# Chang-Tun-Yu/HLS-final-Visual-Odometry

Measured on AMD Instinct MI355X. Metric: stereo frame-pairs/sec (detect+match), KITTI 1241x376; matches bit-exact, higher is better.
Workload: dtype u8; 1 GPU; KITTI 1241x376 stereo quad-match (prev/curr x L/R), default 50x50 bins; noise=0, gpu_max_hw_queues=4, streams_per_gpu=256, frames_in_hbm=8, parallelism=1x independent stream groups

## Files before the change

hls-final-visual-odometry_amd/csrc/kernels_detect.hip:

```cpp
#include "vh_dev.h"
#include "vh_wave.h"
#include <type_traits>

namespace {

__global__ void half_res_kernel(VhImages src, uint8_t *__restrict__ dst, VhGeom g) {
  const int32_t id = blockIdx.z;
  const uint8_t *__restrict__ I = vh_image_ptr(src, id);
  uint8_t *__restrict__ O = dst + (int64_t)id * g.bplm * g.Hm;
  const int32_t u = blockIdx.x * blockDim.x + threadIdx.x;
  const int32_t v = blockIdx.y;
  if (u >= g.bplm) return;
  uint32_t val = 0;
  if (u < g.Wm) {
    const int64_t r0 = (int64_t)(2 * v) * g.bpl + 2 * u, r1 = r0 + g.bpl;
    val = ((uint32_t)I[r0] + I[r0 + 1] + I[r1] + I[r1 + 1]) >> 2;
  }
  O[(int64_t)v * g.bplm + u] = (uint8_t)val;
}

__global__ void __launch_bounds__(256)
detect_nms_kernel(VhImages im, VhGeom g, uint64_t *__restrict__ rec, int32_t *__restrict__ chunk_count) {
  extern __shared__ __attribute__((aligned(16))) uint8_t smem[];
  uint8_t *sI = smem;
  int16_t *sF1 = (int16_t *)(smem + (size_t)g.IH * g.IWp);
  int16_t *sF2 = sF1 + (size_t)g.FH * g.FWp;

  const int32_t id = blockIdx.z;
  const uint8_t *__restrict__ I = vh_image_ptr(im, id);
  const int32_t n = g.n, n1 = n + 1;
  const int32_t bx0 = blockIdx.x * g.tbx, by0 = blockIdx.y * g.tby;
  const int32_t fx0 = VH_MARGIN + bx0 * n1, fy0 = VH_MARGIN + by0 * n1;
  const int32_t ix0 = fx0 - 2, iy0 = fy0 - 2;
  const int32_t tid = threadIdx.x;

  for (int32_t k = tid; k < g.IH * g.IWp; k += 256) {
    const int32_t r = k / g.IWp, c = k - r * g.IWp;
    const int32_t gx = ix0 + c, gy = iy0 + r;
    uint8_t v = 0;
    if (c < g.IW && gx < g.bplm && gy < g.Hm) v = I[(int64_t)gy * g.bplm + gx];
    sI[k] = v;
  }
  __syncthreads();

  {
    const int32_t nseg = max(1, 256 / g.FW);
    const int32_t rows_per = (g.FH + nseg - 1) / nseg;
    for (int32_t task = tid; task < g.FW * nseg; task += 256) {
      const int32_t seg = task / g.FW, cx = task - seg * g.FW;
      const int32_t r0 = seg * rows_per, r1 = min(g.FH, r0 + rows_per);
      if (r0 >= r1) continue;
      int32_t h5[5], h3[5], hc[5], cc[5];
#pragma unroll
      for (int32_t k = 0; k < 4; k++) {
        const uint8_t *p = sI + (size_t)(r0 + k) * g.IWp + cx;
        const int32_t a = p[0], b = p[1], c = p[2], d = p[3], e = p[4];
        h5[k + 1] = a + b + c + d + e; h3[k + 1] = b + c + d; hc[k + 1] = a + b - d - e; cc[k + 1] = c;
      }
      for (int32_t fr = r0; fr < r1; fr++) {
#pragma unroll
        for (int32_t k = 0; k < 4; k++) { h5[k] = h5[k + 1]; h3[k] = h3[k + 1]; hc[k] = hc[k + 1]; cc[k] = cc[k + 1]; }
        const uint8_t *p = sI + (size_t)(fr + 4) * g.IWp + cx;
        const int32_t a = p[0], b = p[1], c = p[2], d = p[3], e = p[4];
        h5[4] = a + b + c + d + e; h3[4] = b + c + d; hc[4] = a + b - d - e; cc[4] = c;
        const int32_t f2 = hc[0] + hc[1] - hc[3] - hc[4];
        const int32_t f1 = -(h5[0] + h5[1] + h5[2] + h5[3] + h5[4]) + 2 * (h3[1] + h3[2] + h3[3]) + 7 * cc[2];
        sF1[(size_t)fr * g.FWp + cx] = (int16_t)f1;
        sF2[(size_t)fr * g.FWp + cx] = (int16_t)f2;
      }
    }
  }
  __syncthreads();

  int32_t *sCnt = (int32_t *)(sF2 + (size_t)g.FH * g.FWp);
  uint32_t *sWork = (uint32_t *)(sCnt + 1);
  uint16_t *sCode = (uint16_t *)(sWork + 4 * g.tbx * g.tby);
  const int32_t nblk_tile = g.tbx * g.tby;
  if (tid == 0) *sCnt = 0;
  for (int32_t k = tid; k < 4 * nblk_tile; k += 256) sCode[k] = VH_NO_CODE;
  __syncthreads();
  const int32_t xlim = (g.Wm - 1 - VH_MARGIN) - fx0, ylim = (g.Hm - 1 - VH_MARGIN) - fy0;
  const int32_t lby = tid / g.tbx, lbx = tid - lby * g.tbx;
  const int32_t bx = bx0 + lbx, by = by0 + lby;
  const bool have_block = tid < nblk_tile && bx < g.nbx && by < g.nby;
  if (have_block) {
    const int32_t fx = n + lbx * n1, fy = n + lby * n1;
    int32_t ex[4], ey[4], ev[4];
    ex[0] = ex[1] = ex[2] = ex[3] = fx;
    ey[0] = ey[1] = ey[2] = ey[3] = fy;
    ev[0] = ev[1] = sF1[(size_t)fy * g.FWp + fx];
    ev[2] = ev[3] = sF2[(size_t)fy * g.FWp + fx];
    for (int32_t j2 = fy; j2 <= fy + n; j2++) {
      for (int32_t i2 = fx; i2 <= fx + n; i2++) {
        int32_t cur = sF1[(size_t)j2 * g.FWp + i2];
        if (cur < ev[0]) { ex[0] = i2; ey[0] = j2; ev[0] = cur; }
        else if (cur > ev[1]) { ex[1] = i2; ey[1] = j2; ev[1] = cur; }
        cur = sF2[(size_t)j2 * g.FWp + i2];
        if (cur < ev[2]) { ex[2] = i2; ey[2] = j2; ev[2] = cur; }
        else if (cur > ev[3]) { ex[3] = i2; ey[3] = j2; ev[3] = cur; }
      }
    }
#pragma unroll
    for (int32_t c = 0; c < 4; c++) {
      const bool pass = (c & 1) ? (ev[c] >= g.tau) : (ev[c] <= -g.tau);
      if (pass) sWork[atomicAdd(sCnt, 1)] = (uint32_t)ex[c] | ((uint32_t)ey[c] << 10) | ((uint32_t)c << 20) | ((uint32_t)tid << 22);
    }
  }
  __syncthreads();
  const int32_t nwork = *sCnt;
  for (int32_t w = tid; w < nwork; w += 256) {
    const uint32_t e = sWork[w];
    const int32_t cx = e & 1023, cy = (e >> 10) & 1023, c = (e >> 20) & 3, owner = e >> 22;
    const int32_t oby = owner / g.tbx, obx = owner - oby * g.tbx;
    const int32_t fx = n + obx * n1, fy = n + oby * n1;
    const int16_t *F = (c < 2) ? sF1 : sF2;
    const bool is_min = (c & 1) == 0;
    const int32_t val = F[(size_t)cy * g.FWp + cx];
    const int32_t jhi = min(cy + n, ylim), ihi = min(cx + n, xlim);
    bool ok = true;
    for (int32_t j2 = cy - n; j2 <= jhi && ok; j2++) {
      for (int32_t i2 = cx - n; i2 <= ihi; i2++) {
        const int32_t cur = F[(size_t)j2 * g.FWp + i2];
        const bool outside = (i2 < fx) | (i2 > fx + n) | (j2 < fy) | (j2 > fy + n);
        if (outside && (is_min ? (cur < val) : (cur > val))) { ok = false; break; }
      }
    }
    if (ok) sCode[owner * 4 + c] = (uint16_t)(((cy - fy) << 6) | (cx - fx));
  }
  __syncthreads();
  if (have_block) {
    uint64_t code = 0;
    int32_t cnt = 0;
#pragma unroll
    for (int32_t c = 0; c < 4; c++) {
      const uint32_t pc = sCode[tid * 4 + c];
      code |= (uint64_t)pc << (16 * c);
      cnt += pc != VH_NO_CODE ? 1 : 0;
    }
    const int32_t blk = by * g.nbx + bx;
    rec[(int64_t)id * g.nblocks + blk] = code;
    if (cnt) atomicAdd(&chunk_count[(int64_t)id * g.nchunks + blk / VH_CHUNK], cnt);
  }
}

#ifdef VH_EMIT_TIMING
__device__ unsigned long long g_emit_t[8];
extern "C" int32_t vh_debug_emit_timing(unsigned long long *out, int32_t reset) {
  if (hipMemcpyFromSymbol(out, HIP_SYMBOL(g_emit_t), sizeof(g_emit_t)) != hipSuccess) return -3;
  if (reset) { unsigned long long z[8] = {0}; z[6] = ~0ull; if (hipMemcpyToSymbol(HIP_SYMBOL(g_emit_t), z, sizeof(z)) != hipSuccess) return -3; }
  return 0;
}
#define VH_TICK_IMPL(k) do { __syncthreads(); if (t_on_) { const unsigned long long now_ = __builtin_readcyclecounter(); atomicAdd(&g_emit_t[k], now_ - t_prev_); t_prev_ = now_; if ((k) == 4) atomicMax(&g_emit_t[7], now_); } } while (0)
#define VH_TICK_INIT_IMPL const bool t_on_ = threadIdx.x == 0 && (blockIdx.x + gridDim.x * (blockIdx.y + gridDim.y * blockIdx.z)) % 61 == 0; unsigned long long t_prev_ = __builtin_readcyclecounter(); if (t_on_) { atomicAdd(&g_emit_t[5], 1ull); atomicMin(&g_emit_t[6], t_prev_); }
#endif
#if defined(VH_EMIT_TIMING) && VH_EMIT_TIMING == 2
#define VH_DTICK(k) VH_TICK_IMPL(k)
#define VH_DTICK_INIT VH_TICK_INIT_IMPL
#else
#define VH_DTICK(k) do { } while (0)
#define VH_DTICK_INIT do { } while (0)
#endif
#if defined(VH_EMIT_TIMING) && VH_EMIT_TIMING != 2
#define VH_ETICK(k) VH_TICK_IMPL(k)
#define VH_ETICK_INIT VH_TICK_INIT_IMPL
#else
#define VH_ETICK(k) do { } while (0)
#define VH_ETICK_INIT do { } while (0)
#endif

#ifdef VH_EXP_DET_STOP
#define VH_DET_STOP(k)                                                                                   \
  if (VH_EXP_DET_STOP == (k) && g.nbx > 0) {                                                              \
    const int32_t sbx = bx0 + tid % T::TBX, sby = by0 + tid / T::TBX;                                     \
    if (sbx < g.nbx && sby < g.nby) rec[(int64_t)id * g.nblocks + sby * g.nbx + sbx] = ~0ull;              \
    return;                                                                                               \
  }
#else
#define VH_DET_STOP(k) do { } while (0)
#endif

template <int N> struct DetTile {
  static constexpr int N1 = N + 1, TBX = 32, TBY = 8;
  static constexpr int FW = TBX * N1 + 2 * N, FH = TBY * N1 + 2 * N;
  static constexpr int IW = FW + 4, IH = FH + 4;
  static constexpr int OFF = (VH_MARGIN - 2) & 3;
  static constexpr int DW = ((IW + 3 + 3) / 4 + 3) / 4 * 4;
  static constexpr int IP = DW * 4;
  static constexpr int NC = DW / 4;
  static constexpr int groups(int px) { return (FW + OFF + px - 1) / px; }
  static constexpr int seg_cost(int px, int s) {
    const int rows = (FH + s - 1) / s, waves = (groups(px) * s + 63) / 64;
    const int hrow = px == 4 ? 28 : 18, vrow = px == 4 ? 26 : 13;
    return groups(px) * s > 256 || rows * (s - 1) >= FH ? (1 << 30) : 1000 * ((rows + 4) * hrow + rows * vrow) + waves;
  }
  static constexpr int best_seg(int px) {
    int b = 1;
    for (int s = 2; s <= 16; s++)
      if (seg_cost(px, s) < seg_cost(px, b)) b = s;
    return b;
  }
#ifdef VH_DET_PX
  static constexpr int PX = VH_DET_PX;
  static constexpr int SEG = VH_DET_SEG;
#else
  static constexpr int PX = seg_cost(2, best_seg(2)) < seg_cost(4, best_seg(4)) ? 2 : 4;
  static constexpr int SEG = best_seg(PX);
#endif
  static constexpr int G = groups(PX);
  static constexpr int FP = PX * G;
  static constexpr int ROWS = (FH + SEG - 1) / SEG;
  static constexpr int BIAS = 8192;
  static_assert((G - 1) * PX / 4 + 1 <= DW - 1, "a group reads the staged dword it starts in and the next one");
  static_assert(G * SEG <= 256, "one lane per (group, row segment)");
  static constexpr int LAST = FH - (SEG - 1) * ROWS;
  static_assert(LAST >= 1, "every segment has rows");
};

template <int N>
__global__ void __launch_bounds__(256)
detect_nms_fast_kernel(VhImages im, VhGeom g, uint64_t *__restrict__ rec, int32_t *__restrict__ chunk_count) {
  using T = DetTile<N>;
  constexpr int N1 = T::N1, WN = 2 * N + 1;
  VH_DET_SETPRIO();
  constexpr int X_BYTES = (T::IH * T::IP > 6144) ? T::IH * T::IP : 6144;
  __shared__ __attribute__((aligned(16))) int16_t sF1[T::FH * T::FP];
  __shared__ __attribute__((aligned(16))) int16_t sF2[T::FH * T::FP];
  __shared__ __attribute__((aligned(16))) uint8_t sX[X_BYTES];
  uint8_t *sI = sX;

  const int32_t id = blockIdx.z, tid = threadIdx.x;
  const uint8_t *__restrict__ I = vh_image_ptr(im, id);
  const int32_t bx0 = blockIdx.x * T::TBX, by0 = blockIdx.y * T::TBY;
  const int32_t fx0 = VH_MARGIN + bx0 * N1, fy0 = VH_MARGIN + by0 * N1;
  const int32_t ix0 = fx0 - 2, iy0 = fy0 - 2;
  const int32_t ax0 = ix0 - T::OFF;
  VH_DTICK_INIT;

  {
    constexpr int NLD = (T::IH * T::NC + 255) / 256;
    typedef uint32_t u32x4a4 __attribute__((ext_vector_type(4), aligned(4)));
    typedef uint32_t u32x4 __attribute__((ext_vector_type(4)));
    const uint32_t last = (uint32_t)g.Hm * (uint32_t)g.bplm - 16u;
    u32x4 stg[NLD];
#pragma unroll
    for (int32_t i = 0; i < NLD; i++) {
      const int32_t k = min(tid + 256 * i, T::IH * T::NC - 1);
      const int32_t r = k / T::NC, c = k - r * T::NC;
      stg[i] = *(const u32x4a4 *)(I + min((uint32_t)(iy0 + r) * (uint32_t)g.bplm + (uint32_t)(ax0 + 16 * c), last));
    }
    __builtin_amdgcn_sched_barrier(0);
#pragma unroll
    for (int32_t i = 0; i < NLD; i++) {
      const int32_t k = tid + 256 * i;
      if (k < T::IH * T::NC) ((u32x4 *)sI)[k] = stg[i];
    }
  }
  __syncthreads();

  VH_DTICK(0);
  VH_DET_STOP(1);
  if (tid < T::G * T::SEG) {
    constexpr int PX = T::PX, NR = PX / 2;
    const int32_t seg = tid / T::G, gq = tid - seg * T::G;
    const int32_t r0 = seg * T::ROWS;
    {
      constexpr uint32_t HB = 512u * 0x00010001u, KB = (uint32_t)T::BIAS * 0x00010001u;
      const uint32_t *p = (const uint32_t *)sI + r0 * T::DW + (gq * PX) / 4;
      const uint32_t sel0 = 0x0c010c00u + ((PX == 2 && (gq & 1)) ? 0x00020002u : 0u);
      uint32_t *o1 = (uint32_t *)sF1 + (r0 * T::FP + PX * gq) / 2, *o2 = (uint32_t *)sF2 + (r0 * T::FP + PX * gq) / 2;
      uint32_t h5[NR][5], h3[NR][5], pc[NR][4], cc[NR][5], hcp[NR], S5[NR];
#pragma unroll
      for (int32_t h = 0; h < NR; h++) S5[h] = 0u;
#pragma unroll
      for (int32_t t = 0; t < T::ROWS + 4; t++) {
        if (t - 4 < T::LAST || r0 + t - 4 < T::FH) {
          const uint32_t A = p[t * T::DW], B = p[t * T::DW + 1];
          uint32_t pk[PX + 3];
#pragma unroll
          for (int32_t k = 0; k < PX + 3; k++) pk[k] = __builtin_amdgcn_perm(B, A, sel0 + (uint32_t)k * 0x00010001u);
          uint32_t n5[NR], n3[NR], nc[NR], nz[NR];
          if (PX == 4) {
            const uint32_t a01 = pk[0] + pk[1], a23 = pk[2] + pk[3], a34 = pk[3] + pk[4], a56 = pk[5] + pk[6];
            n3[0] = a23 + pk[1];             n3[NR - 1] = a34 + pk[5];
            n5[0] = n3[0] + pk[0] + pk[4];   n5[NR - 1] = n3[NR - 1] + pk[2] + pk[6];
            nc[0] = (a01 + HB) - a34;        nc[NR - 1] = (a23 + HB) - a56;
            nz[0] = pk[2];                   nz[NR - 1] = pk[4];
          } else {
            n3[0] = pk[1] + pk[2] + pk[3];
            n5[0] = n3[0] + pk[0] + pk[4];
            nc[0] = ((pk[0] + pk[1]) + HB) - (pk[3] + pk[4]);
            nz[0] = pk[2];
          }
          uint32_t f1[NR], f2[NR];
#pragma unroll
          for (int32_t h = 0; h < NR; h++) {
            const uint32_t old5 = h5[h][0];
#pragma unroll
            for (int32_t k = 0; k < 4; k++) { h5[h][k] = h5[h][k + 1]; h3[h][k] = h3[h][k + 1]; cc[h][k] = cc[h][k + 1]; }
            h5[h][4] = n5[h]; h3[h][4] = n3[h]; cc[h][4] = nz[h];
            S5[h] += n5[h];
            if (t >= 5) S5[h] -= old5;
#pragma unroll
            for (int32_t k = 0; k < 3; k++) pc[h][k] = pc[h][k + 1];
            if (t > 0) pc[h][3] = hcp[h] + nc[h];
            hcp[h] = nc[h];
            if (t >= 4) {
              const uint32_t S3 = h3[h][1] + h3[h][2] + h3[h][3];
              f2[h] = (pc[h][0] + KB) - pc[h][3];
              f1[h] = ((S3 + S3) + (__umul24(cc[h][2], 7u) + KB)) - S5[h];
            }
          }
          if (t >= 4) {
            if (PX == 4) {
              *(uint2 *)(o1 + (t - 4) * (T::FP / 2)) = make_uint2(f1[0], f1[NR - 1]);
              *(uint2 *)(o2 + (t - 4) * (T::FP / 2)) = make_uint2(f2[0], f2[NR - 1]);
            } else {
              o1[(t - 4) * (T::FP / 2)] = f1[0];
              o2[(t - 4) * (T::FP / 2)] = f2[0];
            }
          }
        }
      }
    }
  }
  __syncthreads();
  VH_DTICK(1);
  VH_DET_STOP(2);

  const int32_t xlim = min(max((g.Wm - 1 - VH_MARGIN) - fx0, 0), T::FW - 1);
  const int32_t ylim = min(max((g.Hm - 1 - VH_MARGIN) - fy0, 0), T::FH - 1);
  const int32_t lby = tid / T::TBX, lbx = tid % T::TBX;
  const int32_t bx = bx0 + lbx, by = by0 + lby;
  const bool have_block = bx < g.nbx && by < g.nby;
  const int32_t fx = N + lbx * N1, fy = N + lby * N1;
  uint32_t *sQueue = (uint32_t *)sX;
  uint16_t *sCode = (uint16_t *)(sQueue + 1024);
  __shared__ uint32_t sQueueN;
  if (tid == 0) sQueueN = 0;
  ((uint2 *)sCode)[tid] = make_uint2(VH_NO_CODE * 0x00010001u, VH_NO_CODE * 0x00010001u);
  __syncthreads();
  {
    typedef int16_t i16x2 __attribute__((ext_vector_type(2)));
    const int32_t lane = tid & 63;
    bool cand[4];
    uint32_t ext[4];
#pragma unroll
    for (int32_t plane = 0; plane < 2; plane++) {
      const int16_t *b = (plane ? sF2 : sF1) + fy * T::FP + fx + T::OFF;
      int32_t vn, vx;
      if (N & 1) {
        const i16x2 *bw = (const i16x2 *)b;
        i16x2 mn = bw[0], mx = mn;
#pragma unroll
        for (int32_t j = 0; j < N1; j++) {
#pragma unroll
          for (int32_t d = 0; d < N1 / 2; d++) {
            if (d == 0 && j == 0) continue;
            const i16x2 w = bw[j * (T::FP / 2) + d];
            mn = __builtin_elementwise_min(mn, w);
            mx = __builtin_elementwise_max(mx, w);
          }
        }
        vn = min((int32_t)mn.x, (int32_t)mn.y);
        vx = max((int32_t)mx.x, (int32_t)mx.y);
      } else {
        vn = vx = b[0];
#pragma unroll
        for (int32_t k = 1; k < N1 * N1; k++) {
          const int32_t cur = b[(k / N1) * T::FP + k % N1];
          vn = min(vn, cur);
          vx = max(vx, cur);
        }
      }
      cand[2 * plane] = have_block && vn <= T::BIAS - g.tau;
      cand[2 * plane + 1] = have_block && vx >= T::BIAS + g.tau;
      ext[2 * plane] = (uint32_t)vn;
      ext[2 * plane + 1] = (uint32_t)vx;
    }
    uint64_t bal[4];
#pragma unroll
    for (int32_t t = 0; t < 4; t++) bal[t] = __ballot(cand[t]);
    const uint32_t n0 = (uint32_t)__popcll(bal[0]), n1 = (uint32_t)__popcll(bal[1]);
    const uint32_t add = (n0 + (uint32_t)__popcll(bal[2])) | ((n1 + (uint32_t)__popcll(bal[3])) << 16);
    if (add) {
      uint32_t base = 0;
      if (lane == 0) base = atomicAdd(&sQueueN, add);
      base = __builtin_amdgcn_readfirstlane(base);
#pragma unroll
      for (int32_t t = 0; t < 4; t++) {
        const int32_t mm = t & 1;
        const uint32_t first = ((base >> (16 * mm)) & 0xFFFFu) + (t >= 2 ? (mm ? n1 : n0) : 0u);
        const uint32_t rank = (uint32_t)vh_wave_rank(bal[t]);
        if (cand[t]) sQueue[mm * 512 + first + rank] = (uint32_t)tid | ((uint32_t)t << 8) | (ext[t] << 16);
      }
    }
  }
  __syncthreads();
  VH_DTICK(2);
  VH_DET_STOP(3);
  {
    const int32_t n0 = (int32_t)(sQueueN & 0xFFFFu), ntot = n0 + (int32_t)(sQueueN >> 16);
    const bool unclipped = xlim == T::FW - 1 && ylim == T::FH - 1;
    auto check = [&](auto kind, auto no_clip, int32_t e) {
      const uint32_t q = sQueue[e < n0 ? e : 512 + e - n0];
      const int32_t owner = q & 255, type = (q >> 8) & 3;
      const int32_t ofy = N + (owner / T::TBX) * N1, ofx = N + (owner % T::TBX) * N1;
      const int16_t *F = ((type & 2) ? sF2 : sF1) + T::OFF;
      const int32_t val = (int32_t)(q >> 16);
      const int16_t *bb = F + ofy * T::FP + ofx;
      int32_t pos = (N << 6) | N;
#pragma unroll
      for (int32_t idx = N1 * N1 - 2; idx >= 0; idx--)
        pos = bb[(idx / N1) * T::FP + idx % N1] == val ? (((idx / N1) << 6) | (idx % N1)) : pos;
      const int32_t bj = pos >> 6, bi = pos & 63;
      const int32_t cy = ofy + bj, cx = ofx + bi;
      int32_t v[WN * WN];
      if (decltype(no_clip)::value) {
        const int16_t *w = F + (cy - N) * T::FP + (cx - N);
#pragma unroll
        for (int32_t j = 0; j < WN; j++)
#pragma unroll
          for (int32_t k = 0; k < WN; k++) v[j * WN + k] = w[j * T::FP + k];
      } else {
        int32_t col[WN];
#pragma unroll
        for (int32_t k = 0; k < WN; k++) col[k] = min(cx - N + k, xlim);
#pragma unroll
        for (int32_t j = 0; j < WN; j++) {
          const int16_t *row = F + min(cy - N + j, ylim) * T::FP;
#pragma unroll
          for (int32_t k = 0; k < WN; k++) v[j * WN + k] = row[col[k]];
        }
      }
      const int32_t centre = v[N * WN + N];
      int32_t emin = centre, emax = centre;
#pragma unroll
      for (int32_t k = 0; k < WN * WN; k++) {
        if (decltype(kind)::value != 1) emin = min(emin, v[k]);
        if (decltype(kind)::value != 0) emax = max(emax, v[k]);
      }
      const int32_t ext = decltype(kind)::value == 0 ? emin : decltype(kind)::value == 1 ? emax : ((type & 1) ? emax : emin);
      if (ext == centre) sCode[owner * 4 + type] = (uint16_t)((bj << 6) | bi);
    };
    typedef std::integral_constant<int, 0> KMin;
    typedef std::integral_constant<int, 1> KMax;
    typedef std::integral_constant<int, 2> KBoth;
    for (int32_t e = tid; e < ntot; e += 256) {
      const int32_t e0 = __builtin_amdgcn_readfirstlane(e & ~63);
      if (e0 + 63 < n0) { if (unclipped) check(KMin{}, std::true_type{}, e); else check(KMin{}, std::false_type{}, e); }
      else if (e0 >= n0) { if (unclipped) check(KMax{}, std::true_type{}, e); else check(KMax{}, std::false_type{}, e); }
      else { if (unclipped) check(KBoth{}, std::true_type{}, e); else check(KBoth{}, std::false_type{}, e); }
    }
  }
  __syncthreads();
  VH_DTICK(3);
  VH_DET_STOP(4);
  uint32_t codes[4];
  {
    const uint2 cw = ((const uint2 *)sCode)[tid];
    codes[0] = cw.x & 0xFFFFu; codes[1] = cw.x >> 16; codes[2] = cw.y & 0xFFFFu; codes[3] = cw.y >> 16;
  }

  __shared__ int32_t sChunk[16];
  const int32_t chunk_lo = (by0 * g.nbx + bx0) / VH_CHUNK;
  if (tid < 16) sChunk[tid] = 0;
  __syncthreads();
  if (have_block) {
    int32_t cnt = 0;
#pragma unroll
    for (int32_t c = 0; c < 4; c++) cnt += codes[c] != VH_NO_CODE ? 1 : 0;
    const int32_t blk = by * g.nbx + bx;
    rec[(int64_t)id * g.nblocks + blk] = (uint64_t)(codes[0] | (codes[1] << 16)) | ((uint64_t)(codes[2] | (codes[3] << 16)) << 32);
    if (cnt) atomicAdd(&sChunk[blk / VH_CHUNK - chunk_lo], cnt);
  }
  __syncthreads();
  if (tid < 16 && sChunk[tid]) atomicAdd(&chunk_count[(int64_t)id * g.nchunks + chunk_lo + tid], sChunk[tid]);
  VH_DTICK(4);
}

__constant__ int8_t c_desc_dx[16] = {-3, -3, -1, -1, +3, +3, +1, +1, -1, -1, +1, +1, -5, -5, +5, +5};
__constant__ int8_t c_desc_dy[16] = {-1, +1, -1, +1, -1, +1, -1, +1, -5, +5, -5, +5, -3, +3, -3, +3};


#ifndef VH_EMIT_NF
#define VH_EMIT_NF 2
#endif
__global__ void __launch_bounds__(256)
emit_features_kernel(VhImages im, VhGeom g, const uint64_t *__restrict__ rec,
                     const int32_t *__restrict__ chunk_count, VhSets s) {
  int32_t *__restrict__ feat = s.feat;
  int32_t *__restrict__ count = s.count;
  const int32_t cap = s.cap;
  __shared__ uint32_t sList[4 * VH_CHUNK + 1];
  __shared__ int32_t sWave[4], sWaveP[4];

  const int32_t id = blockIdx.y, chunk = blockIdx.x, tid = threadIdx.x;
  const uint8_t *__restrict__ I = vh_image_ptr(im, id);
  const int32_t set = vh_image_set(im, id);
  const int32_t n1 = g.n + 1;
  VH_DET_SETPRIO();
  VH_ETICK_INIT;

  constexpr int BPL = VH_CHUNK / 256;
  uint32_t clo[BPL], chi[BPL];
  {
    const uint2 *rp = reinterpret_cast<const uint2 *>(rec) + (int64_t)id * g.nblocks;
#pragma unroll
    for (int32_t k = 0; k < BPL; k++) {
      const uint2 c = rp[min(chunk * VH_CHUNK + tid * BPL + k, g.nblocks - 1)];
      clo[k] = c.x; chi[k] = c.y;
    }
  }
  int32_t part = 0;
  for (int32_t k = tid; k < chunk; k += 256) part += chunk_count[(int64_t)id * g.nchunks + k];
  int32_t mine = 0;
#pragma unroll
  for (int32_t k = 0; k < BPL; k++) {
    if (chunk * VH_CHUNK + tid * BPL + k >= g.nblocks) clo[k] = chi[k] = ~0u;
    mine += ((clo[k] & 0xFFFFu) != VH_NO_CODE) + ((clo[k] >> 16) != VH_NO_CODE) + ((chi[k] & 0xFFFFu) != VH_NO_CODE) + ((chi[k] >> 16) != VH_NO_CODE);
  }
  part = vh_wave_sum(part);
  const int32_t incl = vh_wave_scan(mine);
  if ((tid & 63) == 63) { sWave[tid >> 6] = incl; sWaveP[tid >> 6] = part; }
  __syncthreads();
  const int32_t base = sWaveP[0] + sWaveP[1] + sWaveP[2] + sWaveP[3];
  VH_ETICK(0);
  int32_t woff = 0;
  for (int32_t w = 0; w < (tid >> 6); w++) woff += sWave[w];
  const int32_t total = sWave[0] + sWave[1] + sWave[2] + sWave[3];
  int32_t pos = woff + incl - mine;
  {
    const int32_t blk0 = chunk * VH_CHUNK + tid * BPL;
    int32_t by = blk0 / g.nbx, bx = blk0 - by * g.nbx;
    const uint32_t org = (uint32_t)(g.n + VH_MARGIN) * ((1u << 14) + 1u);
#pragma unroll
    for (int32_t k = 0; k < BPL; k++) {
      const uint32_t pxy = org + (uint32_t)(bx * n1) + ((uint32_t)(by * n1) << 14);
#pragma unroll
      for (int32_t q = 0; q < 4; q++) {
        const uint32_t w = (q < 2) ? clo[k] : chi[k];
        const uint32_t pc = (q & 1) ? (w >> 16) : (w & 0xFFFFu);
        const bool ok = pc != VH_NO_CODE;
        const uint32_t e = pxy + (pc & 63u) + ((pc >> 6) << 14) + ((uint32_t)q << 28);
        sList[ok ? pos : 4 * VH_CHUNK] = e;
        pos += ok ? 1 : 0;
      }
      if (++bx == g.nbx) { bx = 0; by++; }
    }
  }
  __syncthreads();
  if (chunk == g.nchunks - 1 && tid == 0) count[set] = base + total;
  VH_ETICK(1);
  const int32_t grp = tid >> 4, k = tid & 15;
  const int32_t dx = c_desc_dx[k], dy = c_desc_dy[k];
  constexpr int NF = VH_EMIT_NF;
  const int32_t prk = min(k, 14) - 7;
  typedef uint32_t u32x4a1 __attribute__((ext_vector_type(4), aligned(1)));
  struct Coords { int32_t fs[NF], us[NF], vs[NF], cs[NF]; bool lives[NF]; };
  auto fetch = [&](int32_t f0, Coords &q, u32x4a1 (&prow)[NF]) {
#pragma unroll
    for (int32_t h = 0; h < NF; h++) {
      q.fs[h] = f0 + 16 * h + grp;
      q.lives[h] = q.fs[h] < total;
      const uint32_t e = sList[q.lives[h] ? q.fs[h] : 0];
      q.us[h] = e & 0x3FFF; q.vs[h] = (e >> 14) & 0x3FFF; q.cs[h] = e >> 28;
#ifdef VH_EXP_NOPATCH
      prow[h] = u32x4a1{(uint32_t)q.us[h], (uint32_t)q.vs[h], 0u, 0u};
#else
      prow[h] = *(const u32x4a1 *)(I + (__umul24((uint32_t)(q.vs[h] + prk), (uint32_t)g.bplm) + (uint32_t)(q.us[h] - 7)));
#endif
    }
  };
  Coords qa, qb;
  u32x4a1 pa[NF], pb[NF];
  if (total > 0) fetch(0, qa, pa);

  constexpr int ROWS_LDS = 64;
  __shared__ int32_t sRow[4 * ROWS_LDS];
  __shared__ __attribute__((aligned(16))) uint16_t sLoc[4 * VH_CHUNK];
  const int32_t blk_first = chunk * VH_CHUNK, blk_last = min(blk_first + VH_CHUNK, g.nblocks) - 1;
  const int32_t v_first = ((blk_first / g.nbx) * n1 + g.n + VH_MARGIN) * g.scale;
  const int32_t v_span = ((blk_last / g.nbx) * n1 + g.n + VH_MARGIN + g.n) * g.scale + g.scale - v_first;
  const bool rows_in_lds = v_span <= ROWS_LDS;
  int32_t *__restrict__ rowh = s.row_hist + (int64_t)set * 4 * s.H;
  auto bin_of_entry = [&](uint32_t e) {
    const int32_t uu = (int32_t)(e & 0x3FFF) * g.scale, vv = (int32_t)((e >> 14) & 0x3FFF) * g.scale, c = e >> 28;
    const int32_t ubin = s.binsize == 1 ? uu : (int32_t)__umulhi((uint32_t)uu, s.inv_binsize);
    const int32_t vbin = s.binsize == 1 ? vv : (int32_t)__umulhi((uint32_t)vv, s.inv_binsize);
    return (c * s.ubn + min(ubin, s.ubn - 1)) * s.vbn + min(vbin, s.vbn - 1);
  };
  const bool have0 = tid < total && base + tid < cap;
  const int32_t b0 = have0 ? bin_of_entry(sList[tid]) : 0;
  int32_t slot0 = 0;
  if (have0) slot0 = atomicAdd(&s.hist[(int64_t)set * s.nbins + b0], 1);
  if (rows_in_lds) {
    for (int32_t k = tid; k < 4 * ROWS_LDS; k += 256) sRow[k] = 0;
    __syncthreads();
    for (int32_t f = tid; f < total && base + f < cap; f += 256) {
      const uint32_t e = sList[f];
      const int32_t vv = (int32_t)((e >> 14) & 0x3FFF) * g.scale, c = e >> 28;
      sLoc[f] = (uint16_t)atomicAdd(&sRow[c * ROWS_LDS + (vv - v_first)], 1);
    }
    __syncthreads();
    for (int32_t k = tid; k < 4 * ROWS_LDS; k += 256) {
      const int32_t cnt = sRow[k], c = k / ROWS_LDS, vv = v_first + k % ROWS_LDS;
      if (cnt) sRow[k] = atomicAdd(&rowh[c * s.H + vv], cnt);
    }
    __syncthreads();
  }
  VH_ETICK(2);
  for (int32_t f = tid; f < total; f += 256) {
    const int32_t fi = base + f;
    if (fi >= cap) break;
    const uint32_t e = sList[f];
    const int32_t vv = (int32_t)((e >> 14) & 0x3FFF) * g.scale, c = e >> 28;
    const int32_t b = f == tid ? b0 : bin_of_entry(e);
    const int32_t rowrel = rows_in_lds ? sRow[c * ROWS_LDS + (vv - v_first)] + (int32_t)sLoc[f] : atomicAdd(&rowh[c * s.H + vv], 1);
    const int32_t slot = f == tid ? slot0 : atomicAdd(&s.hist[(int64_t)set * s.nbins + b], 1);
#ifdef VH_CHECK
    { int32_t sl = slot; VH_CHECK_RANGE(s, 5, sl, 0, s.stage_cap); }
#endif
    if (slot < s.stage_cap) s.stage[((int64_t)set * s.nbins + b) * s.stage_cap + slot] = make_int2(fi, rowrel);
  }

  VH_ETICK(3);
  const int32_t sh = g.scale - 1;
  int32_t *__restrict__ out = feat + (int64_t)set * cap * 12;
  uint32_t *__restrict__ fuv = s.f_uv + (int64_t)set * cap;
  const int32_t gbase = (tid & 63) & ~15, j = (k >= 4) ? (k - 4) : 0;
  const uint32_t m_u = k == 0 ? ~0u : 0u, m_v = k == 1 ? ~0u : 0u, m_c = k == 3 ? ~0u : 0u, m_d = k >= 4 ? ~0u : 0u;
  static_assert(16 * NF * 16 * 16 <= (int)sizeof(sLoc), "the patches reuse sLoc");
  __syncthreads();
  uint32_t *sPatch = (uint32_t *)sLoc + grp * (NF * 64);
  const int32_t rd0 = (dy + 5) * 4 + ((dx + 5) >> 2);
  const uint32_t psel = 0x03020100u + (uint32_t)((dx + 5) & 3) * 0x01010101u;
  auto process = [&](const Coords &q, const u32x4a1 (&prow)[NF]) {
    const int32_t *fs = q.fs, *us = q.us, *vs = q.vs, *cs = q.cs;
    const bool *lives = q.lives;
    uint32_t lo[NF][5], hi[NF][5];
    uint32_t sel[NF];
#pragma unroll
    for (int32_t h = 0; h < NF; h++) sel[h] = psel;
    __builtin_amdgcn_sched_barrier(0);
#pragma unroll
    for (int32_t h = 0; h < NF; h++)
      *(uint4 *)(sPatch + (h * 16 + k) * 4) = make_uint4(prow[h].x, prow[h].y, prow[h].z, prow[h].w);
#pragma unroll
    for (int32_t h = 0; h < NF; h++)
#pragma unroll
      for (int32_t r = 0; r < 5; r++) {
        lo[h][r] = sPatch[h * 64 + rd0 + 4 * r];
        hi[h][r] = sPatch[h * 64 + rd0 + 4 * r + 1];
      }
    __builtin_amdgcn_sched_barrier(0);
#pragma unroll
    for (int32_t h = 0; h < NF; h++) {
      const int32_t u = us[h], v = vs[h];
      uint32_t du_p = 0, du_n = 0, dv_p = 0, dv_n = 0;
#pragma unroll
      for (int32_t r = 0; r < 5; r++) {
        const uint32_t w = __builtin_amdgcn_perm(hi[h][r], lo[h][r], sel[h]);
        const uint32_t w1 = __builtin_amdgcn_perm(hi[h][r], lo[h][r], sel[h] + 0x01010101u);
        const uint32_t sw = (r == 0 || r == 4) ? 1u : (r == 2 ? 6u : 4u);
        du_p = __builtin_amdgcn_udot4(w, sw * 0x00000201u, du_p, false);
        du_n = __builtin_amdgcn_udot4(w1, sw * 0x01020000u, du_n, false);
        if (r != 2) {
          const uint32_t dw = (r == 0 || r == 4) ? 1u : 2u;
          uint32_t &acc = r < 2 ? dv_p : dv_n;
          acc = __builtin_amdgcn_udot4(w, dw * 0x00060401u, acc, false);
          acc = __builtin_amdgcn_udot4(w1, dw * 0x01040000u, acc, false);
        }
      }
      const int32_t a_du = (int32_t)(du_p - du_n), a_dv = (int32_t)(dv_p - dv_n);
      const uint32_t du = (uint32_t)min(255, max(0, (a_du >> 7) + 128));
      const uint32_t dv = (uint32_t)min(255, max(0, (a_dv >> 7) + 128));
      const uint32_t pair = du | (dv << 8);
      const uint32_t plo = __shfl(pair, gbase + 2 * j), phi = __shfl(pair, gbase + 2 * j + 1);
      const uint32_t word = (((uint32_t)u << sh) & m_u) | (((uint32_t)v << sh) & m_v) | ((uint32_t)cs[h] & m_c) | ((plo | (phi << 16)) & m_d);
      const int32_t fi = base + fs[h];
      const bool okf = lives[h] && fi < cap;
      if (okf && k < 12) out[(int64_t)fi * 12 + k] = (int32_t)word;
      if (okf && k == 12) fuv[fi] = (uint32_t)(u << sh) | ((uint32_t)(v << sh) << 16);
    }
  };
  if (total > 0) {
    for (int32_t f0 = 0;; f0 += 32 * NF) {
      const bool more1 = f0 + 16 * NF < total;
      if (more1) fetch(f0 + 16 * NF, qb, pb);
      process(qa, pa);
      if (!more1) break;
      const bool more2 = f0 + 32 * NF < total;
      if (more2) fetch(f0 + 32 * NF, qa, pa);
      process(qb, pb);
      if (!more2) break;
    }
  }
  VH_ETICK(4);
}

__global__ void planes_kernel(const uint8_t *__restrict__ I, int32_t bpl, int32_t H,
                              uint8_t *__restrict__ du, uint8_t *__restrict__ dv,
                              int16_t *__restrict__ f1, int16_t *__restrict__ f2) {
  const int32_t x = blockIdx.x * blockDim.x + threadIdx.x, y = blockIdx.y;
  if (x >= bpl) return;
  const int64_t o = (int64_t)y * bpl + x;
  int32_t r_du = 0, r_dv = 0, r_f1 = 0, r_f2 = 0;
  if (x >= 2 && x <= bpl - 3 && y >= 2 && y <= H - 3) {
    int32_t a_du = 0, a_dv = 0, a_f2 = 0, s5 = 0, s3 = 0, ctr = 0;
#pragma unroll
    for (int32_t r = 0; r < 5; r++) {
      const uint8_t *p = I + (int64_t)(y + r - 2) * bpl + (x - 2);
      const int32_t a = p[0], b = p[1], c = p[2], d = p[3], e = p[4];
      const int32_t sw = (r == 0 || r == 4) ? 1 : (r == 2 ? 6 : 4);
      const int32_t dw = (r == 0) ? 1 : (r == 1 ? 2 : (r == 2 ? 0 : (r == 3 ? -2 : -1)));
      const int32_t cw = (r < 2) ? 1 : (r == 2 ? 0 : -1);
      a_du += sw * (a + 2 * b - 2 * d - e);
      a_dv += dw * (a + 4 * b + 6 * c + 4 * d + e);
      a_f2 += cw * (a + b - d - e);
      s5 += a + b + c + d + e;
      if (r >= 1 && r <= 3) s3 += b + c + d;
      if (r == 2) ctr = c;
    }
    r_du = min(255, max(0, (a_du >> 7) + 128));
    r_dv = min(255, max(0, (a_dv >> 7) + 128));
    r_f2 = a_f2;
    if (x >= 3 && y >= 3) r_f1 = -s5 + 2 * s3 + 7 * ctr;
  }
  if (du) du[o] = (uint8_t)r_du;
  if (dv) dv[o] = (uint8_t)r_dv;
  if (f1) f1[o] = (int16_t)r_f1;
  if (f2) f2[o] = (int16_t)r_f2;
}

}

static bool images_dword_aligned(const VhImages &im, const VhGeom &g) {
  return (g.bplm % 4 == 0) && (im.stride % 4 == 0) && ((uintptr_t)im.base[0] % 4 == 0) &&
         (im.ncam < 2 || (uintptr_t)im.base[1] % 4 == 0);
}

void vh_launch_half_res(const VhImages &src, uint8_t *dst, const VhGeom &g, hipStream_t st) {
  dim3 grid((g.bplm + 255) / 256, g.Hm, src.S * src.ncam);
  hipLaunchKernelGGL(half_res_kernel, grid, dim3(256), 0, st, src, dst, g);
}

void vh_launch_detect_nms(const VhImages &im, const VhGeom &g, uint64_t *rec, int32_t *chunk_count,
                          hipStream_t st) {
  if (g.nblocks <= 0) return;
  if (images_dword_aligned(im, g) && g.n >= 1 && g.n <= 4 && g.nbx <= 2048) {
    dim3 grid((g.nbx + 31) / 32, (g.nby + 7) / 8, im.S * im.ncam);
    switch (g.n) {
      case 1: hipLaunchKernelGGL(detect_nms_fast_kernel<1>, grid, dim3(256), 0, st, im, g, rec, chunk_count); break;
      case 2: hipLaunchKernelGGL(detect_nms_fast_kernel<2>, grid, dim3(256), 0, st, im, g, rec, chunk_count); break;
      case 3: hipLaunchKernelGGL(detect_nms_fast_kernel<3>, grid, dim3(256), 0, st, im, g, rec, chunk_count); break;
      default: hipLaunchKernelGGL(detect_nms_fast_kernel<4>, grid, dim3(256), 0, st, im, g, rec, chunk_count); break;
    }
    return;
  }
  dim3 grid((g.nbx + g.tbx - 1) / g.tbx, (g.nby + g.tby - 1) / g.tby, im.S * im.ncam);
  const size_t lds = (size_t)g.IH * g.IWp + 2 * (size_t)g.FH * g.FWp * sizeof(int16_t) + 4 +
                     (size_t)g.tbx * g.tby * (16 + 8);
  hipLaunchKernelGGL(detect_nms_kernel, grid, dim3(256), lds, st, im, g, rec, chunk_count);
}

void vh_launch_emit_features(const VhImages &im, const VhGeom &g, const uint64_t *rec,
                             const int32_t *chunk_count, const VhSets &s, hipStream_t st) {
  if (g.nblocks <= 0) return;
  dim3 grid(g.nchunks, im.S * im.ncam);
  hipLaunchKernelGGL(emit_features_kernel, grid, dim3(256), 0, st, im, g, rec, chunk_count, s);
}

void vh_launch_planes(const uint8_t *img, int32_t bpl, int32_t H, uint8_t *du, uint8_t *dv,
                      int16_t *f1, int16_t *f2, hipStream_t st) {
  dim3 grid((bpl + 255) / 256, H);
  hipLaunchKernelGGL(planes_kernel, grid, dim3(256), 0, st, img, bpl, H, du, dv, f1, f2);
}
```

Before: 115,500 pairs/s.

## Use signed sdot4 with precomputed per-phase weights in descriptor emit

The descriptor kernel drops the per-row byte permutes and switches to signed dot products. Pixels are biased by XOR 0x80 and multiplied against constant weight words precomputed per sub-word alignment, with the 128 offset folded into the accumulator's initial value. Descriptor pairs are exchanged through LDS instead of shuffles. The f_uv write moves into the binning loop, and addressing is simplified with a per-lane offset and a uniform base. This trims the ALU and shuffle work per feature, at the cost of more weight registers and extra LDS traffic, and it relies on the bias algebra staying bit-exact.

After: 117,100 pairs/s (median of 6 runs). +1.4%, better.

```diff
diff --git a/hls-final-visual-odometry_amd/csrc/kernels_detect.hip b/hls-final-visual-odometry_amd/csrc/kernels_detect.hip
--- a/hls-final-visual-odometry_amd/csrc/kernels_detect.hip
+++ b/hls-final-visual-odometry_amd/csrc/kernels_detect.hip
@@ -480,6 +480,33 @@
 
 __constant__ int8_t c_desc_dx[16] = {-3, -3, -1, -1, +3, +3, +1, +1, -1, -1, +1, +1, -5, -5, +5, +5};
 __constant__ int8_t c_desc_dy[16] = {-1, +1, -1, +1, -1, +1, -1, +1, -5, +5, -5, +5, -3, +3, -3, +3};
+struct DescWeights { uint32_t w[4][16]; };
+constexpr uint64_t desc_taps(int m, int t0, int t1, int t2, int t3, int t4, int a) {
+  return ((uint64_t)(uint8_t)(int8_t)(m * t0) | ((uint64_t)(uint8_t)(int8_t)(m * t1) << 8) | ((uint64_t)(uint8_t)(int8_t)(m * t2) << 16) |
+          ((uint64_t)(uint8_t)(int8_t)(m * t3) << 24) | ((uint64_t)(uint8_t)(int8_t)(m * t4) << 32)) << (8 * a);
+}
+constexpr DescWeights make_desc_weights() {
+  DescWeights d{};
+  const int du_m[3] = {1, 4, 6}, dv_m[4] = {1, 2, -2, -1};
+  for (int a = 0; a < 4; a++) {
+    for (int i = 0; i < 3; i++) {
+      const uint64_t t = desc_taps(du_m[i], 1, 2, 0, -2, -1, a);
+      d.w[a][2 * i] = (uint32_t)t; d.w[a][2 * i + 1] = (uint32_t)(t >> 32);
+    }
+    for (int i = 0; i < 4; i++) {
+      const uint64_t t = desc_taps(dv_m[i], 1, 4, 6, 4, 1, a);
+      d.w[a][6 + 2 * i] = (uint32_t)t; d.w[a][6 + 2 * i + 1] = (uint32_t)(t >> 32);
+    }
+  }
+  return d;
+}
+__constant__ DescWeights c_desc_w = make_desc_weights();
+
+#ifdef VH_EXP_EMIT_STOP
+#define VH_EMIT_STOP(k) if (VH_EXP_EMIT_STOP == (k) && g.nbx > 0) return
+#else
+#define VH_EMIT_STOP(k) do { } while (0)
+#endif
 
 
 #ifndef VH_EMIT_NF
@@ -523,8 +550,9 @@
   const int32_t incl = vh_wave_scan(mine);
   if ((tid & 63) == 63) { sWave[tid >> 6] = incl; sWaveP[tid >> 6] = part; }
   __syncthreads();
-  const int32_t base = sWaveP[0] + sWaveP[1] + sWaveP[2] + sWaveP[3];
+  const int32_t base = __builtin_amdgcn_readfirstlane(sWaveP[0] + sWaveP[1] + sWaveP[2] + sWaveP[3]);
   VH_ETICK(0);
+  VH_EMIT_STOP(1);
   int32_t woff = 0;
   for (int32_t w = 0; w < (tid >> 6); w++) woff += sWave[w];
   const int32_t total = sWave[0] + sWave[1] + sWave[2] + sWave[3];
@@ -551,29 +579,39 @@
   __syncthreads();
   if (chunk == g.nchunks - 1 && tid == 0) count[set] = base + total;
   VH_ETICK(1);
+  VH_EMIT_STOP(2);
   const int32_t grp = tid >> 4, k = tid & 15;
   const int32_t dx = c_desc_dx[k], dy = c_desc_dy[k];
   constexpr int NF = VH_EMIT_NF;
   const int32_t prk = min(k, 14) - 7;
   typedef uint32_t u32x4a1 __attribute__((ext_vector_type(4), aligned(1)));
-  struct Coords { int32_t fs[NF], us[NF], vs[NF], cs[NF]; bool lives[NF]; };
+  const uint32_t lane_off = (uint32_t)(prk * g.bplm - 7);
+  const int32_t last = total - 1;
+  struct Coords { int32_t fs[NF]; uint32_t es[NF]; };
   auto fetch = [&](int32_t f0, Coords &q, u32x4a1 (&prow)[NF]) {
 #pragma unroll
     for (int32_t h = 0; h < NF; h++) {
       q.fs[h] = f0 + 16 * h + grp;
-      q.lives[h] = q.fs[h] < total;
-      const uint32_t e = sList[q.lives[h] ? q.fs[h] : 0];
-      q.us[h] = e & 0x3FFF; q.vs[h] = (e >> 14) & 0x3FFF; q.cs[h] = e >> 28;
+      const uint32_t e = sList[min(q.fs[h], last)];
+      q.es[h] = e;
+      const uint32_t u = e & 0x3FFF, v = (e >> 14) & 0x3FFF;
 #ifdef VH_EXP_NOPATCH
-      prow[h] = u32x4a1{(uint32_t)q.us[h], (uint32_t)q.vs[h], 0u, 0u};
+      prow[h] = u32x4a1{u, v, 0u, 0u};
 #else
-      prow[h] = *(const u32x4a1 *)(I + (__umul24((uint32_t)(q.vs[h] + prk), (uint32_t)g.bplm) + (uint32_t)(q.us[h] - 7)));
+      prow[h] = *(const u32x4a1 *)(I + (__umul24(v, (uint32_t)g.bplm) + u + lane_off));
 #endif
     }
   };
   Coords qa, qb;
   u32x4a1 pa[NF], pb[NF];
   if (total > 0) fetch(0, qa, pa);
+  uint32_t wt[14];
+  {
+    const uint4 *wp = (const uint4 *)c_desc_w.w[(dx + 5) & 3];
+    const uint4 w0 = wp[0], w1 = wp[1], w2 = wp[2], w3 = wp[3];
+    wt[0] = w0.x; wt[1] = w0.y; wt[2] = w0.z; wt[3] = w0.w; wt[4] = w1.x; wt[5] = w1.y; wt[6] = w1.z; wt[7] = w1.w;
+    wt[8] = w2.x; wt[9] = w2.y; wt[10] = w2.z; wt[11] = w2.w; wt[12] = w3.x; wt[13] = w3.y;
+  }
 
   constexpr int ROWS_LDS = 64;
   __shared__ int32_t sRow[4 * ROWS_LDS];
@@ -609,11 +647,14 @@
     __syncthreads();
   }
   VH_ETICK(2);
+  const int32_t sh = g.scale - 1;
+  uint32_t *__restrict__ fuv = s.f_uv + (int64_t)set * cap;
   for (int32_t f = tid; f < total; f += 256) {
     const int32_t fi = base + f;
     if (fi >= cap) break;
     const uint32_t e = sList[f];
     const int32_t vv = (int32_t)((e >> 14) & 0x3FFF) * g.scale, c = e >> 28;
+    fuv[fi] = ((e & 0x3FFF) << sh) | ((((e >> 14) & 0x3FFF) << sh) << 16);
     const int32_t b = f == tid ? b0 : bin_of_entry(e);
     const int32_t rowrel = rows_in_lds ? sRow[c * ROWS_LDS + (vv - v_first)] + (int32_t)sLoc[f] : atomicAdd(&rowh[c * s.H + vv], 1);
     const int32_t slot = f == tid ? slot0 : atomicAdd(&s.hist[(int64_t)set * s.nbins + b], 1);
@@ -624,27 +665,23 @@
   }
 
   VH_ETICK(3);
-  const int32_t sh = g.scale - 1;
-  int32_t *__restrict__ out = feat + (int64_t)set * cap * 12;
-  uint32_t *__restrict__ fuv = s.f_uv + (int64_t)set * cap;
-  const int32_t gbase = (tid & 63) & ~15, j = (k >= 4) ? (k - 4) : 0;
-  const uint32_t m_u = k == 0 ? ~0u : 0u, m_v = k == 1 ? ~0u : 0u, m_c = k == 3 ? ~0u : 0u, m_d = k >= 4 ? ~0u : 0u;
+  VH_EMIT_STOP(3);
+  char *__restrict__ outb = (char *)(feat + (int64_t)set * cap * 12) + (int64_t)base * 48;
+  const int32_t lim = k < 12 ? min(total, cap - base) : 0;
+  const uint32_t hdr_off = k == 0 ? 0u : (k == 1 ? 14u : 28u), hdr_bits = k < 2 ? 14u : (k == 3 ? 4u : 0u), hdr_sh = k < 2 ? (uint32_t)sh : 0u;
+  const bool is_hdr = k < 4;
+  const int32_t j = is_hdr ? 0 : k - 4;
   static_assert(16 * NF * 16 * 16 <= (int)sizeof(sLoc), "the patches reuse sLoc");
   __syncthreads();
   uint32_t *sPatch = (uint32_t *)sLoc + grp * (NF * 64);
+  typedef uint16_t u16alias __attribute__((may_alias));
   const int32_t rd0 = (dy + 5) * 4 + ((dx + 5) >> 2);
-  const uint32_t psel = 0x03020100u + (uint32_t)((dx + 5) & 3) * 0x01010101u;
   auto process = [&](const Coords &q, const u32x4a1 (&prow)[NF]) {
-    const int32_t *fs = q.fs, *us = q.us, *vs = q.vs, *cs = q.cs;
-    const bool *lives = q.lives;
     uint32_t lo[NF][5], hi[NF][5];
-    uint32_t sel[NF];
-#pragma unroll
-    for (int32_t h = 0; h < NF; h++) sel[h] = psel;
     __builtin_amdgcn_sched_barrier(0);
 #pragma unroll
     for (int32_t h = 0; h < NF; h++)
-      *(uint4 *)(sPatch + (h * 16 + k) * 4) = make_uint4(prow[h].x, prow[h].y, prow[h].z, prow[h].w);
+      *(uint4 *)(sPatch + (h * 16 + k) * 4) = make_uint4(prow[h].x ^ 0x80808080u, prow[h].y ^ 0x80808080u, prow[h].z ^ 0x80808080u, prow[h].w ^ 0x80808080u);
 #pragma unroll
     for (int32_t h = 0; h < NF; h++)
 #pragma unroll
@@ -655,32 +692,24 @@
     __builtin_amdgcn_sched_barrier(0);
 #pragma unroll
     for (int32_t h = 0; h < NF; h++) {
-      const int32_t u = us[h], v = vs[h];
-      uint32_t du_p = 0, du_n = 0, dv_p = 0, dv_n = 0;
+      int32_t a_du = 128 << 7, a_dv = 128 << 7;
 #pragma unroll
       for (int32_t r = 0; r < 5; r++) {
-        const uint32_t w = __builtin_amdgcn_perm(hi[h][r], lo[h][r], sel[h]);
-        const uint32_t w1 = __builtin_amdgcn_perm(hi[h][r], lo[h][r], sel[h] + 0x01010101u);
-        const uint32_t sw = (r == 0 || r == 4) ? 1u : (r == 2 ? 6u : 4u);
-        du_p = __builtin_amdgcn_udot4(w, sw * 0x00000201u, du_p, false);
-        du_n = __builtin_amdgcn_udot4(w1, sw * 0x01020000u, du_n, false);
+        const int32_t wu = (r == 0 || r == 4) ? 0 : (r == 2 ? 4 : 2);
+        a_du = __builtin_amdgcn_sdot4((int32_t)lo[h][r], (int32_t)wt[wu], a_du, false);
+        a_du = __builtin_amdgcn_sdot4((int32_t)hi[h][r], (int32_t)wt[wu + 1], a_du, false);
         if (r != 2) {
-          const uint32_t dw = (r == 0 || r == 4) ? 1u : 2u;
-          uint32_t &acc = r < 2 ? dv_p : dv_n;
-          acc = __builtin_amdgcn_udot4(w, dw * 0x00060401u, acc, false);
-          acc = __builtin_amdgcn_udot4(w1, dw * 0x01040000u, acc, false);
+          const int32_t wv = 6 + 2 * (r < 2 ? r : r - 1);
+          a_dv = __builtin_amdgcn_sdot4((int32_t)lo[h][r], (int32_t)wt[wv], a_dv, false);
+          a_dv = __builtin_amdgcn_sdot4((int32_t)hi[h][r], (int32_t)wt[wv + 1], a_dv, false);
         }
       }
-      const int32_t a_du = (int32_t)(du_p - du_n), a_dv = (int32_t)(dv_p - dv_n);
-      const uint32_t du = (uint32_t)min(255, max(0, (a_du >> 7) + 128));
-      const uint32_t dv = (uint32_t)min(255, max(0, (a_dv >> 7) + 128));
-      const uint32_t pair = du | (dv << 8);
-      const uint32_t plo = __shfl(pair, gbase + 2 * j), phi = __shfl(pair, gbase + 2 * j + 1);
-      const uint32_t word = (((uint32_t)u << sh) & m_u) | (((uint32_t)v << sh) & m_v) | ((uint32_t)cs[h] & m_c) | ((plo | (phi << 16)) & m_d);
-      const int32_t fi = base + fs[h];
-      const bool okf = lives[h] && fi < cap;
-      if (okf && k < 12) out[(int64_t)fi * 12 + k] = (int32_t)word;
-      if (okf && k == 12) fuv[fi] = (uint32_t)(u << sh) | ((uint32_t)(v << sh) << 16);
+      const uint32_t du = (uint32_t)min(255, max(0, a_du >> 7));
+      const uint32_t dv = (uint32_t)min(255, max(0, a_dv >> 7));
+      ((u16alias *)(sPatch + h * 64))[k] = (uint16_t)(du | (dv << 8));
+      const uint32_t hdr = __builtin_amdgcn_ubfe(q.es[h], hdr_off, hdr_bits) << hdr_sh;
+      const uint32_t desc = sPatch[h * 64 + j];
+      if (q.fs[h] < lim) *(uint32_t *)(outb + (__umul24((uint32_t)q.fs[h], 48u) + 4u * (uint32_t)k)) = is_hdr ? hdr : desc;
     }
   };
   if (total > 0) {
```
